# uber-research/deep-neuroevolution

Hardware: AMD Instinct MI355X
Metric: env-steps/sec/generation (Frostbite ES pop 5000) (higher is better)
Workload: dtype f32

## Files before the change

### deep-neuroevolution_amd/csrc/forward.h

```cpp
#pragma once
#include <hip/hip_runtime.h>
#include <stdint.h>
#include <type_traits>
#include <utility>

namespace dne {

struct Layout {
    int kind, nact, P;
    int c1w, c1b, bn1b, bn1g, c2w, c2b, bn2b, bn2g, fcw, fcb, bn3b, bn3g, ow, ob;
    int c3w, c3b;
};

__device__ __forceinline__ int opt_off(int off) { return off < 0 ? 0 : off; }
__device__ __forceinline__ float opt_bias(int off, float v) { return off < 0 ? 0.0f : v; }
__device__ __forceinline__ float opt_gamma(int off, float v) { return off < 0 ? 1.0f : v; }

constexpr int TT_MAX = 48;
struct TailTable {
    int n;
    int member[TT_MAX];
    int slot[TT_MAX];
    float scale[TT_MAX];
    long long off[TT_MAX];
// ... 2319 lines not shown
        for (int v = 0; v < NV; v++) all_done = all_done && A.done[member[v]] != 0;
        if (all_done) return;
    }
    DNE_PHASE(2, 0);
    const int kbeg = 968 * sl;
    const int beg = wv == 0 ? 0 : FC_SUB0 + FC_SUBN * (wv - 1);
    const int ng = (wv == 0 ? FC_SUB0 : FC_SUBN) / 4;
    const size_t o0 = (size_t)(kbeg + beg + r) * 256 + cb * 64 + c4 * 4;
    const float *ep = item_eps<TT>(A, first) + L.fcw + o0, *tp = item_base<TT>(A, first) + L.fcw + o0;
    float yv[NV][2], s2[NV][2], h2[NV][2];
#pragma unroll
    for (int v = 0; v < NV; v++)
#pragma unroll
        for (int j = 0; j < 2; j++) {
            const int i = tid + 512 * j, ch = (kbeg + i) & 31;
            const bool in = i < 968;
            yv[v][j] = in ? y2[(size_t)member[v] * 3872 + kbeg + i] : 0.0f;
            s2[v][j] = HAS_BN && in ? A.bn[(size_t)member[v] * 608 + 32 + ch] : 1.0f;
            h2[v][j] = HAS_BN && in ? A.bn[(size_t)member[v] * 608 + 64 + ch] : 0.0f;
        }
    __builtin_amdgcn_sched_barrier(0);
    f4u e[D];
    f4a t[D];
#pragma unroll
    for (int i = 0; i < D; i++) {
        if (NOISE) e[i] = *(const f4u *)(ep + (size_t)i * 1024);
        t[i] = *(const f4a *)(tp + (size_t)i * 1024);
    }
    __builtin_amdgcn_sched_barrier(0);
#pragma unroll
    for (int v = 0; v < NV; v++)
#pragma unroll
        for (int j = 0; j < 2; j++) {
            const int i = tid + 512 * j;
            if (i < 968) {
                float x = yv[v][j];
                if (HAS_BN) {
                    x = x * s2[v][j];
                    x = x + h2[v][j];
                }
                S.xs[v][i] = x > 0.0f ? x : 0.0f;
            }
        }
    __syncthreads();
    DNE_PHASE(2, 1);
    float acc[NV][4];
#pragma unroll
    for (int v = 0; v < NV; v++)
#pragma unroll
        for (int q = 0; q < 4; q++) acc[v][q] = 0.0f;
#pragma unroll
    for (int g = 0; g < FC_SUB0 / 4; g++) {
        if (g < ng) {
            const int slot = g % D;
            f4a x4[NV];
            float w[NV][4];
#pragma unroll
            for (int v = 0; v < NV; v++) {
                x4[v] = *(const f4a *)&S.xs[v][beg + 4 * g];
#pragma unroll
                for (int q = 0; q < 4; q++) {
                    float pv = NOISE ? scale[v] * e[slot][q] : 0.0f;
                    w[v][q] = NOISE ? t[slot][q] + pv : t[slot][q];
                }
            }
            if (g + D < ng) {
                if (NOISE) e[slot] = *(const f4u *)(ep + (size_t)(g + D) * 1024);
                t[slot] = *(const f4a *)(tp + (size_t)(g + D) * 1024);
            }
            if constexpr (NV == 2) {
                asm("s_nop 1\n\t"
                        "v_fmac_f32_dpp %[a00], %[w00], %[x00] quad_perm:[0,0,0,0] row_mask:0xf bank_mask:0xf\n\t"
                        "v_fmac_f32_dpp %[a10], %[w10], %[x10] quad_perm:[0,0,0,0] row_mask:0xf bank_mask:0xf\n\t"
                        "v_fmac_f32_dpp %[a01], %[w01], %[x00] quad_perm:[0,0,0,0] row_mask:0xf bank_mask:0xf\n\t"
                        "v_fmac_f32_dpp %[a11], %[w11], %[x10] quad_perm:[0,0,0,0] row_mask:0xf bank_mask:0xf\n\t"
                        "v_fmac_f32_dpp %[a02], %[w02], %[x00] quad_perm:[0,0,0,0] row_mask:0xf bank_mask:0xf\n\t"
                        "v_fmac_f32_dpp %[a12], %[w12], %[x10] quad_perm:[0,0,0,0] row_mask:0xf bank_mask:0xf\n\t"
                        "v_fmac_f32_dpp %[a03], %[w03], %[x00] quad_perm:[0,0,0,0] row_mask:0xf bank_mask:0xf\n\t"
                        "v_fmac_f32_dpp %[a13], %[w13], %[x10] quad_perm:[0,0,0,0] row_mask:0xf bank_mask:0xf\n\t"
                        "v_fmac_f32_dpp %[a00], %[w00], %[x01] quad_perm:[1,1,1,1] row_mask:0xf bank_mask:0xf\n\t"
                        "v_fmac_f32_dpp %[a10], %[w10], %[x11] quad_perm:[1,1,1,1] row_mask:0xf bank_mask:0xf\n\t"
                        "v_fmac_f32_dpp %[a01], %[w01], %[x01] quad_perm:[1,1,1,1] row_mask:0xf bank_mask:0xf\n\t"
                        "v_fmac_f32_dpp %[a11], %[w11], %[x11] quad_perm:[1,1,1,1] row_mask:0xf bank_mask:0xf\n\t"
                        "v_fmac_f32_dpp %[a02], %[w02], %[x01] quad_perm:[1,1,1,1] row_mask:0xf bank_mask:0xf\n\t"
                        "v_fmac_f32_dpp %[a12], %[w12], %[x11] quad_perm:[1,1,1,1] row_mask:0xf bank_mask:0xf\n\t"
                        "v_fmac_f32_dpp %[a03], %[w03], %[x01] quad_perm:[1,1,1,1] row_mask:0xf bank_mask:0xf\n\t"
                        "v_fmac_f32_dpp %[a13], %[w13], %[x11] quad_perm:[1,1,1,1] row_mask:0xf bank_mask:0xf\n\t"
                        "v_fmac_f32_dpp %[a00], %[w00], %[x02] quad_perm:[2,2,2,2] row_mask:0xf bank_mask:0xf\n\t"
                        "v_fmac_f32_dpp %[a10], %[w10], %[x12] quad_perm:[2,2,2,2] row_mask:0xf bank_mask:0xf\n\t"
                        "v_fmac_f32_dpp %[a01], %[w01], %[x02] quad_perm:[2,2,2,2] row_mask:0xf bank_mask:0xf\n\t"
                        "v_fmac_f32_dpp %[a11], %[w11], %[x12] quad_perm:[2,2,2,2] row_mask:0xf bank_mask:0xf\n\t"
                        "v_fmac_f32_dpp %[a02], %[w02], %[x02] quad_perm:[2,2,2,2] row_mask:0xf bank_mask:0xf\n\t"
                        "v_fmac_f32_dpp %[a12], %[w12], %[x12] quad_perm:[2,2,2,2] row_mask:0xf bank_mask:0xf\n\t"
                        "v_fmac_f32_dpp %[a03], %[w03], %[x02] quad_perm:[2,2,2,2] row_mask:0xf bank_mask:0xf\n\t"
                        "v_fmac_f32_dpp %[a13], %[w13], %[x12] quad_perm:[2,2,2,2] row_mask:0xf bank_mask:0xf\n\t"
                        "v_fmac_f32_dpp %[a00], %[w00], %[x03] quad_perm:[3,3,3,3] row_mask:0xf bank_mask:0xf\n\t"
                        "v_fmac_f32_dpp %[a10], %[w10], %[x13] quad_perm:[3,3,3,3] row_mask:0xf bank_mask:0xf\n\t"
                        "v_fmac_f32_dpp %[a01], %[w01], %[x03] quad_perm:[3,3,3,3] row_mask:0xf bank_mask:0xf\n\t"
                        "v_fmac_f32_dpp %[a11], %[w11], %[x13] quad_perm:[3,3,3,3] row_mask:0xf bank_mask:0xf\n\t"
                        "v_fmac_f32_dpp %[a02], %[w02], %[x03] quad_perm:[3,3,3,3] row_mask:0xf bank_mask:0xf\n\t"
                        "v_fmac_f32_dpp %[a12], %[w12], %[x13] quad_perm:[3,3,3,3] row_mask:0xf bank_mask:0xf\n\t"
                        "v_fmac_f32_dpp %[a03], %[w03], %[x03] quad_perm:[3,3,3,3] row_mask:0xf bank_mask:0xf\n\t"
                        "v_fmac_f32_dpp %[a13], %[w13], %[x13] quad_perm:[3,3,3,3] row_mask:0xf bank_mask:0xf\n\t"
                        : [a00] "+v"(acc[0][0]), [a01] "+v"(acc[0][1]), [a02] "+v"(acc[0][2]), [a03] "+v"(acc[0][3]), [a10] "+v"(acc[1][0]), [a11] "+v"(acc[1][1]), [a12] "+v"(acc[1][2]), [a13] "+v"(acc[1][3])
                        : [w00] "v"(w[0][0]), [w01] "v"(w[0][1]), [w02] "v"(w[0][2]), [w03] "v"(w[0][3]), [w10] "v"(w[1][0]), [w11] "v"(w[1][1]), [w12] "v"(w[1][2]), [w13] "v"(w[1][3]), [x00] "v"(x4[0][0]), [x01] "v"(x4[0][1]), [x02] "v"(x4[0][2]), [x03] "v"(x4[0][3]), [x10] "v"(x4[1][0]), [x11] "v"(x4[1][1]), [x12] "v"(x4[1][2]), [x13] "v"(x4[1][3]));
            } else {
                asm("s_nop 1\n\t"
                        "v_fmac_f32_dpp %[a00], %[w00], %[x00] quad_perm:[0,0,0,0] row_mask:0xf bank_mask:0xf\n\t"
                        "v_fmac_f32_dpp %[a01], %[w01], %[x00] quad_perm:[0,0,0,0] row_mask:0xf bank_mask:0xf\n\t"
                        "v_fmac_f32_dpp %[a02], %[w02], %[x00] quad_perm:[0,0,0,0] row_mask:0xf bank_mask:0xf\n\t"
                        "v_fmac_f32_dpp %[a03], %[w03], %[x00] quad_perm:[0,0,0,0] row_mask:0xf bank_mask:0xf\n\t"
                        "v_fmac_f32_dpp %[a00], %[w00], %[x01] quad_perm:[1,1,1,1] row_mask:0xf bank_mask:0xf\n\t"
                        "v_fmac_f32_dpp %[a01], %[w01], %[x01] quad_perm:[1,1,1,1] row_mask:0xf bank_mask:0xf\n\t"
                        "v_fmac_f32_dpp %[a02], %[w02], %[x01] quad_perm:[1,1,1,1] row_mask:0xf bank_mask:0xf\n\t"
                        "v_fmac_f32_dpp %[a03], %[w03], %[x01] quad_perm:[1,1,1,1] row_mask:0xf bank_mask:0xf\n\t"
                        "v_fmac_f32_dpp %[a00], %[w00], %[x02] quad_perm:[2,2,2,2] row_mask:0xf bank_mask:0xf\n\t"
                        "v_fmac_f32_dpp %[a01], %[w01], %[x02] quad_perm:[2,2,2,2] row_mask:0xf bank_mask:0xf\n\t"
                        "v_fmac_f32_dpp %[a02], %[w02], %[x02] quad_perm:[2,2,2,2] row_mask:0xf bank_mask:0xf\n\t"
                        "v_fmac_f32_dpp %[a03], %[w03], %[x02] quad_perm:[2,2,2,2] row_mask:0xf bank_mask:0xf\n\t"
                        "v_fmac_f32_dpp %[a00], %[w00], %[x03] quad_perm:[3,3,3,3] row_mask:0xf bank_mask:0xf\n\t"
                        "v_fmac_f32_dpp %[a01], %[w01], %[x03] quad_perm:[3,3,3,3] row_mask:0xf bank_mask:0xf\n\t"
                        "v_fmac_f32_dpp %[a02], %[w02], %[x03] quad_perm:[3,3,3,3] row_mask:0xf bank_mask:0xf\n\t"
                        "v_fmac_f32_dpp %[a03], %[w03], %[x03] quad_perm:[3,3,3,3] row_mask:0xf bank_mask:0xf\n\t"
                        : [a00] "+v"(acc[0][0]), [a01] "+v"(acc[0][1]), [a02] "+v"(acc[0][2]), [a03] "+v"(acc[0][3])
                        : [w00] "v"(w[0][0]), [w01] "v"(w[0][1]), [w02] "v"(w[0][2]), [w03] "v"(w[0][3]), [x00] "v"(x4[0][0]), [x01] "v"(x4[0][1]), [x02] "v"(x4[0][2]), [x03] "v"(x4[0][3]));
            }
        }
    }
    if (r == 0) {
#pragma unroll
        for (int v = 0; v < NV; v++)
#pragma unroll
            for (int q = 0; q < 4; q++) S.comb[wv][v][c4 * 4 + q] = acc[v][q];
    }
    DNE_PHASE(2, 2);
    __syncthreads();
    DNE_PHASE(2, 3);
    if (tid < NV * 64) {
        const int v = tid >> 6, col = tid & 63;
        float f = S.comb[0][v][col];
#pragma unroll
        for (int i = 1; i < 8; i++) f = f + S.comb[i][v][col];
        y3t[((size_t)(first.member + v) * 4 + sl) * 256 + cb * 64 + col] = f;
    }
    DNE_PHASE(2, 4);
}

template <int NV, bool HAS_BN, bool NOISE = true>
__global__ __launch_bounds__(512) void k_fc_tail(FwdArgs A, const int *__restrict__ list, const float *__restrict__ y2,
                                                 float *__restrict__ y3t ) {
    __shared__ TailFcLds<NV> S;
    const int item = blockIdx.x >> 4, sl = (blockIdx.x >> 2) & 3, cb = blockIdx.x & 3;
    if (A.tt.n > 0) fc_tail_body<NV, HAS_BN, true, NOISE>(S, A, list, item, sl, cb, y2, y3t);
    else fc_tail_body<NV, HAS_BN, false, NOISE>(S, A, list, item, sl, cb, y2, y3t);
}

template <int NV, bool HAS_BN>
__global__ __launch_bounds__(256) void k_fc_cols(FwdArgs A, const int *__restrict__ list, const float *__restrict__ y2,
                                                 float *__restrict__ y3t ) {
    __shared__ float xs[4][NV][968];
    const int tid = threadIdx.x, wv = tid >> 6, lane = tid & 63;
    const Layout &L = A.L;
    const int item = blockIdx.x >> 2, cq = blockIdx.x & 3;
    const int g = list ? list[item] : item;
    int member[NV];
    float scale[NV];
#pragma unroll
    for (int v = 0; v < NV; v++) { member[v] = g * NV + v; scale[v] = A.m_scale[member[v]]; }
    if (A.done) {
        bool all_done = true;
#pragma unroll
        for (int v = 0; v < NV; v++) all_done = all_done && A.done[member[v]] != 0;
        if (all_done) return;
    }
    const int64_t off = A.m_off[member[0]];
    const float *base = A.bases + (size_t)A.m_slot[member[0]] * A.base_stride;
    const int col = cq * 64 + lane;
    const int kbeg = 968 * wv;
    const float *eps = A.noise + off + L.fcw + (size_t)kbeg * 256 + col;
    const float *th = base + L.fcw + (size_t)kbeg * 256 + col;
    constexpr int RB = 40, R0 = FC_SUB0 - 3 * RB;
    static_assert(R0 == 8 && FC_SUBN == 3 * RB && R0 + 24 * RB == 968, "batches must end on the sub-slice boundaries");
    float e0[R0], t0[R0], e_cur[RB], t_cur[RB], e_nxt[RB], t_nxt[RB];
#pragma unroll
    for (int i = 0; i < R0; i++) { e0[i] = eps[(size_t)i * 256]; t0[i] = th[(size_t)i * 256]; }
#pragma unroll
    for (int i = 0; i < RB; i++) { e_cur[i] = eps[(size_t)(R0 + i) * 256]; t_cur[i] = th[(size_t)(R0 + i) * 256]; }
    {
        float yv[NV][16], s2[NV], h2[NV];
        const int ch = (kbeg + lane) & 31;
#pragma unroll
        for (int v = 0; v < NV; v++) {
            s2[v] = HAS_BN ? A.bn[(size_t)member[v] * 608 + 32 + ch] : 1.0f;
            h2[v] = HAS_BN ? A.bn[(size_t)member[v] * 608 + 64 + ch] : 0.0f;
#pragma unroll
            for (int j = 0; j < 16; j++) {
                const int i = lane + 64 * j;
                yv[v][j] = i < 968 ? y2[(size_t)member[v] * 3872 + kbeg + i] : 0.0f;
            }
        }
#pragma unroll
        for (int v = 0; v < NV; v++)
#pragma unroll
            for (int j = 0; j < 16; j++) {
                const int i = lane + 64 * j;
                if (i < 968) {
                    float t = yv[v][j];
                    if (HAS_BN) {
                        t = t * s2[v];
                        t = t + h2[v];
                    }
                    xs[wv][v][i] = t > 0.0f ? t : 0.0f;
                }
            }
    }
    __syncthreads();
    float acc[NV], fold[NV];
#pragma unroll
    for (int v = 0; v < NV; v++) acc[v] = fold[v] = 0.0f;
#pragma unroll
    for (int i = 0; i < R0; i++) {
#pragma unroll
        for (int v = 0; v < NV; v++) {
            float pv = scale[v] * e0[i];
            const float w = t0[i] + pv;
            acc[v] = __builtin_fmaf(xs[wv][v][i], w, acc[v]);
        }
    }
    for (int bt = 0; bt < 24; bt++) {
        if (bt + 1 < 24) {
#pragma unroll
            for (int i = 0; i < RB; i++) {
                e_nxt[i] = eps[(size_t)(R0 + (bt + 1) * RB + i) * 256];
                t_nxt[i] = th[(size_t)(R0 + (bt + 1) * RB + i) * 256];
            }
        }
#pragma unroll
        for (int i = 0; i < RB; i++) {
#pragma unroll
            for (int v = 0; v < NV; v++) {
                float pv = scale[v] * e_cur[i];
                const float w = t_cur[i] + pv;
                acc[v] = __builtin_fmaf(xs[wv][v][R0 + bt * RB + i], w, acc[v]);
            }
        }
#pragma unroll
        for (int i = 0; i < RB; i++) { e_cur[i] = e_nxt[i]; t_cur[i] = t_nxt[i]; }
        if (bt % 3 == 2) {
#pragma unroll
            for (int v = 0; v < NV; v++) { fold[v] = bt == 2 ? acc[v] : fold[v] + acc[v]; acc[v] = 0.0f; }
        }
    }
#pragma unroll
    for (int v = 0; v < NV; v++) y3t[((size_t)member[v] * 4 + wv) * 256 + col] = fold[v];
}

template <int NV, bool HAS_BN, bool NOISE>
__global__ __launch_bounds__(256) void k_fc_sub(FwdArgs A, const int *__restrict__ list, int n_groups, int spw ,
                                                int prio, const float *__restrict__ y2, float *__restrict__ y3s ) {
    constexpr int W = 8;
    const int tid = threadIdx.x, wv = tid >> 6, lane = tid & 63;
    const unsigned voff = lane * 16;
    const Layout &L = A.L;
    const int upg = 32 / spw;
    if (prio == 3) __builtin_amdgcn_s_setprio(3);
    else if (prio == 2) __builtin_amdgcn_s_setprio(2);
    else if (prio == 1) __builtin_amdgcn_s_setprio(1);
    for (int w = uni(blockIdx.x * 4 + wv); w < n_groups * upg; w += gridDim.x * 4) {
    const int gi = w / upg, j = w - gi * upg;
    const int g = uni(list ? list[gi] : gi);
    if (A.done) {
        int all_done = 1;
#pragma unroll
        for (int v = 0; v < NV; v++) all_done &= uni(A.done[g * NV + v]) != 0;
        if (all_done) continue;
    }
    const int m0 = g * NV;
    const long long off = uni64(A.m_off[m0]);
    const float *base = A.bases + (size_t)uni(A.m_slot[m0]) * A.base_stride + L.fcw;
    const float *eps = A.noise + off + L.fcw;
    float scale[NV];
#pragma unroll
    for (int v = 0; v < NV; v++) scale[v] = A.m_scale[m0 + v];
    for (int s = 0; s < spw; s++) {
        const int u = j * spw + s, q = u >> 3, i = u & 7;
        const int nrows = i == 0 ? FC_SUB0 : FC_SUBN;
        const int R0 = 968 * q + (i == 0 ? 0 : FC_SUB0 + FC_SUBN * (i - 1));
        float xa[NV], xb[NV];
        {
            const int ra = R0 + lane, rb = R0 + min(64 + lane, nrows - 1);
#pragma unroll
            for (int v = 0; v < NV; v++) {
                float a = y2[(size_t)(m0 + v) * 3872 + ra], b = y2[(size_t)(m0 + v) * 3872 + rb];
                if (HAS_BN) {
                    const float *bn = A.bn + (size_t)(m0 + v) * 608;
                    a = a * bn[32 + (ra & 31)]; a = a + bn[64 + (ra & 31)];
                    b = b * bn[32 + (rb & 31)]; b = b + bn[64 + (rb & 31)];
                }
                xa[v] = a > 0.0f ? a : 0.0f;
                xb[v] = b > 0.0f ? b : 0.0f;
                asm volatile("" : "+v"(xa[v]), "+v"(xb[v]));
            }
        }
        const float *tnext = base + (size_t)R0 * 256;
        const float *enext = eps + (size_t)R0 * 256;
        f32x2 acc[NV][2];
#pragma unroll
        for (int v = 0; v < NV; v++) acc[v][0] = acc[v][1] = f32x2{0.0f, 0.0f};
        f32x4 t[W], e[NOISE ? W : 1];
#pragma unroll
        for (int r = 0; r < W; r++) t[r] = f32x4{0.f, 0.f, 0.f, 0.f};
#pragma unroll
        for (int r = 0; r < (NOISE ? W : 1); r++) e[r] = f32x4{0.f, 0.f, 0.f, 0.f};
        constexpr int PENDING = (W - 1) * (NOISE ? 2 : 1);
        auto refill = [&](auto ii) {
            constexpr int I = decltype(ii)::value;
            if constexpr (NOISE) {
                if constexpr (NV == 2) gload4_after<(I % 4) * 1024>(e[I], voff, enext + (I / 4) * 1024, acc[0][0], acc[0][1], acc[1][0], acc[1][1]);
                else gload4_after<(I % 4) * 1024>(e[I], voff, enext + (I / 4) * 1024, acc[0][0], acc[0][1]);
                gload4<(I % 4) * 1024>(t[I], voff, tnext + (I / 4) * 1024);
            } else {
                if constexpr (NV == 2) gload4_after<(I % 4) * 1024>(t[I], voff, tnext + (I / 4) * 1024, acc[0][0], acc[0][1], acc[1][0], acc[1][1]);
                else gload4_after<(I % 4) * 1024>(t[I], voff, tnext + (I / 4) * 1024, acc[0][0], acc[0][1]);
            }
        };
        static_for<W>(refill);
        tnext += W * 256; enext += W * 256;
        const int nb = nrows / W;
        for (int b = 0; b < nb; b++) {
            const int li = (b & 7) * W;
            float xs[NV];
#pragma unroll
            for (int v = 0; v < NV; v++) xs[v] = b < 8 ? xa[v] : xb[v];
            auto one = [&](auto ii) {
                constexpr int I = decltype(ii)::value;
                wait_rows<PENDING>(t[I], e[NOISE ? I : 0]);
                const f32x2 tlo = {t[I][0], t[I][1]}, thi = {t[I][2], t[I][3]};
#pragma unroll
                for (int v = 0; v < NV; v++) {
                    const float x = lane_bcast(xs[v], li + I);
                    const f32x2 xx = {x, x};
                    f32x2 wl = tlo, wh = thi;
                    if constexpr (NOISE) {
                        const f32x2 sc = {scale[v], scale[v]}, elo = {e[I][0], e[I][1]}, ehi = {e[I][2], e[I][3]};
                        const f32x2 pl = sc * elo, ph = sc * ehi;
                        wl = tlo + pl; wh = thi + ph;
                    }
                    acc[v][0] = __builtin_elementwise_fma(xx, wl, acc[v][0]);
                    acc[v][1] = __builtin_elementwise_fma(xx, wh, acc[v][1]);
                }
                __builtin_amdgcn_sched_barrier(0);
                refill(ii);
                __builtin_amdgcn_sched_barrier(0);
            };
            static_for<W>(one);
            tnext += W * 256; enext += W * 256;
        }
#pragma unroll
        for (int r = 0; r < W; r++) wait_rows<0>(t[r], e[NOISE ? r : 0]);
#pragma unroll
        for (int v = 0; v < NV; v++) {
            const f4a o = {acc[v][0][0], acc[v][0][1], acc[v][1][0], acc[v][1][1]};
            *(f4a *)(y3s + ((size_t)(m0 + v) * 32 + u) * 256 + lane * 4) = o;
        }
    }
    }
}

template <int NV, bool HAS_BN>
__global__ __launch_bounds__(256) void k_out(FwdArgs A, const int *__restrict__ list, const float *__restrict__ y3t,
                                            float *__restrict__ y3, int32_t *__restrict__ actions,
                                            float *__restrict__ logits_out) {
    __shared__ float red[4][NV][OUT_NA];
    __shared__ float lg[NV][32];
    const int tid = threadIdx.x, wv = tid >> 6, lane = tid & 63;
    const Layout &L = A.L;
    const int g = list ? list[blockIdx.x] : blockIdx.x;
    const int nact = L.nact;
    if (A.done) {
        bool all_done = true;
#pragma unroll
        for (int v = 0; v < NV; v++) all_done = all_done && A.done[g * NV + v] != 0;
        if (all_done) return;
    }
    DNE_WG_BEGIN;
    const int m0 = g * NV;
    const int64_t off = A.m_off[m0];
    const float *base = A.bases + (size_t)A.m_slot[m0] * A.base_stride;
    const float *eps = A.noise + off;
    float sc[NV], x3[NV];
#pragma unroll
    for (int v = 0; v < NV; v++) sc[v] = A.m_scale[m0 + v];
    const float fb_t = opt_bias(L.fcb, base[opt_off(L.fcb) + tid]), fb_e = opt_bias(L.fcb, eps[opt_off(L.fcb) + tid]);
#pragma unroll
    for (int v = 0; v < NV; v++) {
        const int m = m0 + v;
        float t = fc_combine(y3t, m, tid, A.sub_sums != 0);
        float pvb = sc[v] * fb_e;
        const float fb = fb_t + pvb;
        t = t + fb;
        y3[(size_t)m * 256 + tid] = t;
        if (HAS_BN) {
            t = t * A.bn[(size_t)m * 608 + 96 + tid];
            t = t + A.bn[(size_t)m * 608 + 352 + tid];
        }
        x3[v] = t > 0.0f ? t : 0.0f;
    }
    {
        float p[NV][OUT_NA];
        out_products<NV>(p, x3, base + L.ow + tid * nact, eps + L.ow + tid * nact, sc, nact);
        out_wave_sums<NV>(p, nact, red[wv], lane);
    }
    __syncthreads();
    if (tid < NV * nact) {
        const int v = tid / nact, a = tid % nact;
        const float s01 = red[0][v][a] + red[1][v][a];
        const float s23 = red[2][v][a] + red[3][v][a];
        const float t = s01 + s23;
        float pv = A.m_scale[m0 + v] * eps[L.ob + a];
        const float bias = base[L.ob + a] + pv;
        lg[v][a] = t + bias;
    }
    __syncthreads();
    if (tid < NV) {
        const int v = tid, m = m0 + v;
        int best = 0;
        for (int a = 1; a < nact; a++)
            if (lg[v][a] > lg[v][best]) best = a;
        actions[m] = best;
        if (logits_out)
            for (int a = 0; a < nact; a++) logits_out[(size_t)m * nact + a] = lg[v][a];
    }
    DNE_WG_END(2);
}

template <int C>
__global__ __launch_bounds__(256) void k_bn_finalize(FwdArgs A, int member0, int n_local, int F, const float *__restrict__ fr,
                                                     int npos, int bn_off, int bias_off, int beta_off, int gamma_off) {
    const int i = blockIdx.x * 256 + threadIdx.x, mloc = i / C, c = i % C;
    if (mloc >= n_local) return;
    const int member = member0 + mloc;
    const float *p = fr + (size_t)mloc * F * 2 * C + c;
    float S = 0.0f, Q = 0.0f;
    for (int n = 0; n < F; n++) {
        S = S + p[(size_t)n * 2 * C];
        Q = Q + p[(size_t)n * 2 * C + C];
    }
    const float count = (float)(F * npos);
    const float *base = A.bases + (size_t)A.m_slot[member] * A.base_stride;
    const float *eps = A.noise + A.m_off[member];
    const float sc = A.m_scale[member];
    float pbias = sc * eps[opt_off(bias_off) + c];
    const float bias = opt_bias(bias_off, base[opt_off(bias_off) + c] + pbias);
    const float m = S / count;
    const float mean = bias + m;
    const float q1 = Q / count;
    const float mm = m * m;
    float var = q1 - mm;
    var = var > 0.0f ? var : 0.0f;
    float pb = sc * eps[beta_off + c];
    const float beta = base[beta_off + c] + pb;
    float pg = sc * eps[opt_off(gamma_off) + c];
    const float gamma = opt_gamma(gamma_off, base[opt_off(gamma_off) + c] + pg);
    const float inv = 1.0f / sqrtf(var + 1e-3f);
    const float s = inv * gamma;
    const float ms = mean * s;
    A.bn[(size_t)member * 608 + bn_off + c] = s;
    A.bn[(size_t)member * 608 + bn_off + C + c] = beta - ms;
    A.bn_mom[(size_t)member * 608 + bn_off + c] = mean;
    A.bn_mom[(size_t)member * 608 + bn_off + C + c] = var;
}

__global__ __launch_bounds__(256) void k_bn3_rows(FwdArgs A, int member0, int F, const float *__restrict__ y) {
    const int mloc = blockIdx.x, member = member0 + mloc, j = threadIdx.x;
    const Layout &L = A.L;
    const float *ym = y + (size_t)mloc * F * 256 + j;
    const float count = (float)F;
    float tot = 0.0f;
    for (int n = 0; n < F; n++) tot = tot + (0.0f + ym[(size_t)n * 256]);
    const float mean = tot / count;
    float totq = 0.0f;
    for (int n = 0; n < F; n++) {
        const float d = ym[(size_t)n * 256] - mean;
        totq = totq + __builtin_fmaf(d, d, 0.0f);
    }
    const float var = totq / count;
    const float *base = A.bases + (size_t)A.m_slot[member] * A.base_stride;
    const float *eps = A.noise + A.m_off[member];
    const float sc = A.m_scale[member];
    float pb = sc * eps[L.bn3b + j];
    const float beta = base[L.bn3b + j] + pb;
    float pg = sc * eps[opt_off(L.bn3g) + j];
    const float gamma = opt_gamma(L.bn3g, base[opt_off(L.bn3g) + j] + pg);
    const float inv = 1.0f / sqrtf(var + 1e-3f);
    const float s = inv * gamma;
    const float ms = mean * s;
    A.bn[(size_t)member * 608 + 96 + j] = s;
    A.bn[(size_t)member * 608 + 352 + j] = beta - ms;
    A.bn_mom[(size_t)member * 608 + 96 + j] = mean;
    A.bn_mom[(size_t)member * 608 + 352 + j] = var;
}

}
```

Measured before the change: 2.712 million.

## Skip zero ReLU activation rows in FC weight streaming via ballot compaction

After ReLU, the FC-layer kernel builds a wave-wide ballot mask of input rows that are nonzero for any member. It then streams only those weight and noise rows, picking each row index with ctz and broadcasting its activation with readlane, and skips the tile entirely when no row is live. This is meant to cut global memory traffic for the sparse post-ReLU activations. In exchange it adds scalar bookkeeping and data-dependent row addresses in the pipelined refill, which replace the previous fixed-stride loads.

```diff
diff --git a/deep-neuroevolution_amd/csrc/forward.h b/deep-neuroevolution_amd/csrc/forward.h
--- a/deep-neuroevolution_amd/csrc/forward.h
+++ b/deep-neuroevolution_amd/csrc/forward.h
@@ -2645,43 +2645,62 @@
                 asm volatile("" : "+v"(xa[v]), "+v"(xb[v]));
             }
         }
-        const float *tnext = base + (size_t)R0 * 256;
-        const float *enext = eps + (size_t)R0 * 256;
+        bool live_a = false, live_b = false;
+#pragma unroll
+        for (int v = 0; v < NV; v++) { live_a = live_a || xa[v] != 0.0f; live_b = live_b || xb[v] != 0.0f; }
+        unsigned long long ma = __builtin_amdgcn_ballot_w64(live_a);
+        unsigned long long mb = __builtin_amdgcn_ballot_w64(live_b) & (~0ull >> (128 - nrows));
+        const int n = __builtin_popcountll(ma) + __builtin_popcountll(mb);
+        const float *tbase = base + (size_t)R0 * 256;
+        const float *ebase = eps + (size_t)R0 * 256;
         f32x2 acc[NV][2];
 #pragma unroll
         for (int v = 0; v < NV; v++) acc[v][0] = acc[v][1] = f32x2{0.0f, 0.0f};
+        if (n != 0) {
         f32x4 t[W], e[NOISE ? W : 1];
 #pragma unroll
         for (int r = 0; r < W; r++) t[r] = f32x4{0.f, 0.f, 0.f, 0.f};
 #pragma unroll
         for (int r = 0; r < (NOISE ? W : 1); r++) e[r] = f32x4{0.f, 0.f, 0.f, 0.f};
         constexpr int PENDING = (W - 1) * (NOISE ? 2 : 1);
+        int xs[W][NV];
+        int rlast = 0;
         auto refill = [&](auto ii) {
             constexpr int I = decltype(ii)::value;
+            const bool in_a = ma != 0;
+            const unsigned long long m = in_a ? ma : mb;
+            const bool ok = m != 0;
+            const int r = ok ? __builtin_ctzll(m | (1ull << 63)) + (in_a ? 0 : 64) : rlast;
+            const unsigned long long rest = m & (m - 1);
+            ma = in_a ? rest : 0ull;
+            mb = in_a ? mb : rest;
+            rlast = r;
+#pragma unroll
+            for (int v = 0; v < NV; v++) {
+                const int x0 = __builtin_amdgcn_readlane(__float_as_int(xa[v]), r & 63), x1 = __builtin_amdgcn_readlane(__float_as_int(xb[v]), r & 63);
+                xs[I][v] = !ok ? 0 : r < 64 ? x0 : x1;
+            }
+            const float *trow = tbase + (size_t)r * 256;
             if constexpr (NOISE) {
-                if constexpr (NV == 2) gload4_after<(I % 4) * 1024>(e[I], voff, enext + (I / 4) * 1024, acc[0][0], acc[0][1], acc[1][0], acc[1][1]);
-                else gload4_after<(I % 4) * 1024>(e[I], voff, enext + (I / 4) * 1024, acc[0][0], acc[0][1]);
-                gload4<(I % 4) * 1024>(t[I], voff, tnext + (I / 4) * 1024);
+                const float *erow = ebase + (size_t)r * 256;
+                if constexpr (NV == 2) gload4_after<0>(e[I], voff, erow, acc[0][0], acc[0][1], acc[1][0], acc[1][1]);
+                else gload4_after<0>(e[I], voff, erow, acc[0][0], acc[0][1]);
+                gload4<0>(t[I], voff, trow);
             } else {
-                if constexpr (NV == 2) gload4_after<(I % 4) * 1024>(t[I], voff, tnext + (I / 4) * 1024, acc[0][0], acc[0][1], acc[1][0], acc[1][1]);
-                else gload4_after<(I % 4) * 1024>(t[I], voff, tnext + (I / 4) * 1024, acc[0][0], acc[0][1]);
+                if constexpr (NV == 2) gload4_after<0>(t[I], voff, trow, acc[0][0], acc[0][1], acc[1][0], acc[1][1]);
+                else gload4_after<0>(t[I], voff, trow, acc[0][0], acc[0][1]);
             }
         };
         static_for<W>(refill);
-        tnext += W * 256; enext += W * 256;
-        const int nb = nrows / W;
+        const int nb = (n + W - 1) / W;
         for (int b = 0; b < nb; b++) {
-            const int li = (b & 7) * W;
-            float xs[NV];
-#pragma unroll
-            for (int v = 0; v < NV; v++) xs[v] = b < 8 ? xa[v] : xb[v];
             auto one = [&](auto ii) {
                 constexpr int I = decltype(ii)::value;
                 wait_rows<PENDING>(t[I], e[NOISE ? I : 0]);
                 const f32x2 tlo = {t[I][0], t[I][1]}, thi = {t[I][2], t[I][3]};
 #pragma unroll
                 for (int v = 0; v < NV; v++) {
-                    const float x = lane_bcast(xs[v], li + I);
+                    const float x = __int_as_float(xs[I][v]);
                     const f32x2 xx = {x, x};
                     f32x2 wl = tlo, wh = thi;
                     if constexpr (NOISE) {
@@ -2697,10 +2716,10 @@
                 __builtin_amdgcn_sched_barrier(0);
             };
             static_for<W>(one);
-            tnext += W * 256; enext += W * 256;
         }
 #pragma unroll
         for (int r = 0; r < W; r++) wait_rows<0>(t[r], e[NOISE ? r : 0]);
+        }
 #pragma unroll
         for (int v = 0; v < NV; v++) {
             const f4a o = {acc[v][0][0], acc[v][0][1], acc[v][1][0], acc[v][1][1]};
```

After: 2.737 million, median of 6. No clear change (+0.9%).
